# wangsibovictor/fora

Hardware: AMD Instinct MI355X
Metric: SSPPR queries/sec at eps=0.5 (higher is better)
Workload: dtype u64 fixed-point 2^-62 (f64 at the boundary)

## Files before the change

### fora_amd/csrc/fora_hip.hip

```cpp
#include "fora_kernels.h"
#include "fora_team.h"
#include "fora_bwd.h"
#include "../../include/fora_hip.h"

#include <algorithm>
#include <cmath>
#include <cstdio>
#include <cstdlib>
#include <cstring>
#include <string>
#include <vector>

using namespace fora;

struct fora_ctx;
static int build_hub_copy(fora_ctx *c, const int64_t *row_ptr, const int32_t *col);
static int build_quad_copies(fora_ctx *c);
namespace {

struct EvPair {
    hipEvent_t a, b;
    int kind;
};

// ... 16 lines not shown
    int64_t xb = 0, ax = 0, wx = 0;
    int64_t tail = -1;
    int64_t tail_always = 0;
    int64_t select_compact = -1;
    int64_t rounds = 1;
    int64_t round_div = 4;
    int64_t defer = 0;
    int64_t defer_min = 0;
    int64_t team = -1;
    int64_t team_size = 0;
    int64_t team_tail = -1;
    int64_t team_xcd = 1;
    int64_t team_max = 0;
    int64_t team_hubs = 1024;
    int64_t tail_hubs = 1;
    int64_t team_log = -1;
    int64_t slot_major = -1;
    int64_t acc_group = 0;
    int64_t team_abort_level = 0;
    int64_t team_timeout_ms = 500;
    int64_t team_coop = 0;
    int64_t topk_bk_div = 16;
    int64_t quads = 1;
    int64_t pipeline = 0;
    int64_t profile = 1;
    int64_t grid = 2048;
    int64_t bwd_lds_cap = BWD_CAP_DEFAULT;
    int64_t bwd_chunk = 0;
};
static const struct { const char *name; int64_t Tunables::*field; bool layout; } OPTIONS[] = {
    {"direct", &Tunables::direct, true}, {"force_wide", &Tunables::force_wide, true}, {"pass_bins", &Tunables::pass_bins, true},
    {"no_split", &Tunables::no_split, true}, {"no_compact", &Tunables::no_compact, false}, {"walk_dg", &Tunables::walk_dg, false}, {"dg_hubs", &Tunables::dg_hubs, false}, {"hubs", &Tunables::hubs, true}, {"hubs_wide", &Tunables::hubs_wide, true}, {"hub_min", &Tunables::hub_min, false}, {"bkcap", &Tunables::bkcap, true},
    {"ovcap", &Tunables::ovcap, true}, {"tiny", &Tunables::tiny, false}, {"xb", &Tunables::xb, false}, {"ax", &Tunables::ax, false},
    {"wx", &Tunables::wx, false}, {"tail", &Tunables::tail, false}, {"tail_always", &Tunables::tail_always, false},
    {"select_compact", &Tunables::select_compact, false}, {"pipeline", &Tunables::pipeline, false}, {"team", &Tunables::team, true}, {"team_size", &Tunables::team_size, true}, {"team_tail", &Tunables::team_tail, false}, {"team_xcd", &Tunables::team_xcd, false}, {"team_max", &Tunables::team_max, true}, {"team_hubs", &Tunables::team_hubs, true}, {"team_log", &Tunables::team_log, false}, {"topk_bk_div", &Tunables::topk_bk_div, true}, {"quads", &Tunables::quads, false}, {"team_timeout_ms", &Tunables::team_timeout_ms, false}, {"team_abort_level", &Tunables::team_abort_level, false}, {"acc_group", &Tunables::acc_group, false}, {"slot_major", &Tunables::slot_major, false}, {"team_coop", &Tunables::team_coop, false}, {"tail_hubs", &Tunables::tail_hubs, false}, {"rounds", &Tunables::rounds, false}, {"defer", &Tunables::defer, true}, {"defer_min", &Tunables::defer_min, false}, {"round_div", &Tunables::round_div, false},
    {"profile", &Tunables::profile, false}, {"grid", &Tunables::grid, false},
    {"bwd_lds_cap", &Tunables::bwd_lds_cap, false}, {"bwd_chunk", &Tunables::bwd_chunk, false},
};
static bool schedule_option(const char *name) {
    return !strcmp(name, "rounds") || !strcmp(name, "round_div") || !strcmp(name, "defer") || !strcmp(name, "defer_min");
}
static Tunables tunables_from_env() {
    Tunables t;
    for (const auto &o : OPTIONS) {
        if (schedule_option(o.name)) continue;
        std::string env = "FORA_HIP_";
        for (const char *p = o.name; *p; p++) env += (char)toupper((unsigned char)*p);
        if (const char *e = getenv(env.c_str())) if (*e) t.*(o.field) = atoll(e);
    }
    return t;
// ... 29 lines not shown
    uint32_t *d_dg_perm = nullptr, *d_dg_inv = nullptr, *d_dg_colp = nullptr, *d_dg_rec = nullptr, *d_dg_invb = nullptr;
    uint8_t *d_dg_T = nullptr;
    WalkDG dg{};
    uint32_t *d_colt = nullptr, *d_team_off = nullptr, *d_team_n2l = nullptr, *d_team_l2n = nullptr;
    uint32_t *d_team_hubtgt = nullptr;
    uint32_t team_H = 0, team_hubs_opt = 0;
    uint16_t *d_team_rlog_id = nullptr; uint64_t *d_team_rlog_val = nullptr; uint32_t team_rlog_cap = 0;
    uint64_t *d_team_rowl = nullptr, *d_team_rsvl = nullptr;
    uint16_t *d_team_deg16 = nullptr;
    uint32_t *d_team_rowq = nullptr;
    uint32_t team_T = 0, team_R = 0, team_force = 0;
    bool team_checked = false, team_wanted = false;
    double dangling_frac = 0;
    uint64_t team_cap = 0;
    uint32_t *d_team_msg = nullptr;
    uint64_t *d_team_inct = nullptr;
    unsigned long long *d_team_cnt = nullptr;
    uint32_t *d_team_ctl = nullptr;
    uint32_t team_n = 0;
    bool team_dirty = false;
    bool hub_for_team = false;
    bool team_timeout_seen = false;
    int team_suspend = 0;
    uint64_t team_fallbacks = 0;
    int team_fit = -1;
    bool team_coop_ok = false;
    bool team_coop_failed = false;

    bool have_params = false;
    double alpha = 0.2, epsilon = 0.5, rmax_scale = 1.0, rmax = 0, omega = 0;
// ... 126 lines not shown
void free_index(fora_ctx *c) {
    dfree(c->d_rw_idx); dfree(c->d_idx_off); dfree(c->d_idx_cnt);
    c->idx_len = 0; c->have_index = false;
}
void free_workspace(fora_ctx *c) {
    dfree(c->d_residue); dfree(c->d_ppr); dfree(c->d_wl[0]); dfree(c->d_wl[1]); dfree(c->d_scratch);
    dfree(c->d_counters); dfree(c->d_qs); dfree(c->d_src); dfree(c->d_err);
    dfree(c->d_ppr2); dfree(c->d_cursor); c->cursor_epoch = 0; dfree(c->d_active); dfree(c->d_above); dfree(c->d_sel_thr); dfree(c->d_topk_ids); dfree(c->d_topk_sc);
    dfree(c->d_upper); dfree(c->d_lower); dfree(c->d_filter); dfree(c->d_fail); dfree(c->d_round_walks);
    dfree(c->d_lb_sc); dfree(c->d_lb_ids); c->lb_cap = 0;
    dfree(c->d_nz_counts);
    c->topk_cap = 0;
    dfree(c->d_fl[0]); dfree(c->d_fl[1]); dfree(c->d_fl_count); dfree(c->d_inc_tab[0]); dfree(c->d_inc_tab[1]); dfree(c->d_ov_w); dfree(c->d_ov_inc); dfree(c->d_ov_count); dfree(c->d_ov_bin);
    dfree(c->d_bk_w); dfree(c->d_bk_inc); dfree(c->d_bk_count); dfree(c->d_wit_count); dfree(c->d_sw); dfree(c->d_tile_ctr);
    dfree(c->d_dbm); dfree(c->d_dflag); dfree(c->d_dl); dfree(c->d_hubsum);
    dfree(c->d_team_msg); dfree(c->d_team_inct); dfree(c->d_team_rsvl); dfree(c->d_team_rlog_id); dfree(c->d_team_rlog_val); dfree(c->d_team_cnt); dfree(c->d_team_ctl); c->team_n = 0; c->team_fit = -1;
    if (c->h_flc) (void)hipHostFree(c->h_flc);
    c->h_flc = nullptr;
    if (c->h_pinned) (void)hipHostFree(c->h_pinned);
    c->h_pinned = nullptr;
    if (c->h_qs_pin) (void)hipHostFree(c->h_qs_pin);
    c->h_qs_pin = nullptr;
    if (c->h_steps_pin) (void)hipHostFree(c->h_steps_pin);
    c->h_steps_pin = nullptr;
    c->B = 0;
    c->B_memcap = 0;
}

constexpr size_t N_COUNTERS = 2 * (size_t)(MAX_LEVELS + 2) + 2;
static uint32_t slab_grid_x(const fora_ctx *c, int nq) {
    const int64_t nchunk = ((int64_t)c->n + BLOCK - 1) / BLOCK;
// ... 224 lines not shown
               c->wit_cap >= pe.wits && c->bk_cap == pe.bk_cap && c->sub == pe.sub;
    };
    {
        int need = c->batch_req > 0 ? c->batch_req : std::min(want_slots > 0 ? want_slots : 1024, 1024);
        if (c->batch_req == 0 && c->B > 0 && c->B_memcap > 0) need = std::min(need, c->B_memcap);
        if (keepable(need)) { const WsPlan pe = plan_workspace(c, omega_hint, c->B); return ensure_row_split(c, pe.nbins, pe.pbins); }
    }
    int B = c->batch_req > 0 ? c->batch_req : 0;
    if (B == 0) {
        free_workspace(c);
        size_t fr = 0, tot = 0;
        HIPCHK(c, hipMemGetInfo(&fr, &tot));
        uint64_t budget = (uint64_t)(fr * (c->opt_.pipeline == 1 ? 0.4 : 0.75));
        if (c->team_T) {
            const uint64_t T = c->team_T, nt = std::max<uint64_t>(1, (uint64_t)c->prop.multiProcessorCount * TEAM_WGS_PER_CU / T);
            const uint64_t team_bytes = nt * (2 * c->team_cap * 4 + 3 * T * (c->team_R + 64 + c->team_H) * 8 + T * (10ull << 17) + 2 * T * T * 8);
            budget -= std::min<uint64_t>(budget / 2, team_bytes);
        }
        B = (int)std::min<uint64_t>(1024, std::max<uint64_t>(1, budget / p.per_slot));
    }
    B = std::max(1, B);
    const int memcap = B;
    if (want_slots > 0 && c->batch_req == 0) B = std::min(B, std::max(want_slots, 1));
    p = plan_workspace(c, omega_hint, B);
    const uint64_t scratch = (uint64_t)B * p.scratch;
    free_workspace(c);
    const uint64_t slab = (uint64_t)B * n;
    HIPCHK(c, hipMalloc(&c->d_residue, slab * 8));
    HIPCHK(c, hipMalloc(&c->d_ppr, slab * 8));
    if (p.binned) {
        HIPCHK(c, hipMalloc(&c->d_fl[0], slab * 4));
// ... 12 lines not shown
        HIPCHK(c, hipMalloc(&c->d_bk_count, (size_t)B * p.pbins * p.sub * 4));
        HIPCHK(c, hipHostMalloc(&c->h_flc, (size_t)FLC_RING * B * 4 * CSTRIDE));
        c->dbm_words = (uint32_t)((uint64_t)p.nbins << (bin_shift(c) - 6));
        HIPCHK(c, hipMalloc(&c->d_dbm, 2 * (size_t)B * c->dbm_words * 8));
        HIPCHK(c, hipMalloc(&c->d_dflag, 2 * (size_t)B * p.nbins * 4));
        if (c->opt_.defer > 0) HIPCHK(c, hipMalloc(&c->d_dl, 2 * slab * 4));
        if (c->hubs && c->hub_shift == bin_shift(c)) HIPCHK(c, hipMalloc(&c->d_hubsum, (size_t)B * p.sub * c->hubs * 8));
        if (c->team_T) {
            const uint32_t T = c->team_T;
            uint32_t nteams = std::max<uint32_t>(1, (uint32_t)c->prop.multiProcessorCount * TEAM_WGS_PER_CU / T);
            if (c->opt_.team_max > 0) nteams = std::min<uint32_t>(nteams, (uint32_t)c->opt_.team_max);
            size_t fr = 0, tot = 0;
            HIPCHK(c, hipMemGetInfo(&fr, &tot));
            c->team_rlog_cap = 1u << 17;
            auto per_team_bytes = [&](uint32_t logcap) {
                return 2 * c->team_cap * 4 + 3 * (uint64_t)T * (c->team_R + 64 + c->team_H) * 8 + (uint64_t)T * logcap * 10 + 2 * (uint64_t)T * T * 8;
            };
            while (c->team_rlog_cap > 1024 && per_team_bytes(c->team_rlog_cap) > fr / 4) c->team_rlog_cap /= 2;
            const uint64_t per_team = per_team_bytes(c->team_rlog_cap);
            nteams = (uint32_t)std::max<uint64_t>(1, std::min<uint64_t>(nteams, (uint64_t)(fr / 2) / std::max<uint64_t>(1, per_team)));
            HIPCHK(c, hipMalloc(&c->d_team_msg, (size_t)nteams * 2 * c->team_cap * 4 + 64 + diag::TEAM_MSG_PROBE_WORDS * 4));
            HIPCHK(c, hipMalloc(&c->d_team_inct, (size_t)nteams * 2 * T * (c->team_R + 64 + c->team_H) * 8));
            HIPCHK(c, hipMalloc(&c->d_team_rsvl, (size_t)nteams * T * c->team_R * 8));
            HIPCHK(c, hipMemset(c->d_team_rsvl, 0, (size_t)nteams * T * c->team_R * 8));
            HIPCHK(c, hipMalloc(&c->d_team_rlog_id, (size_t)nteams * T * c->team_rlog_cap * 2));
            HIPCHK(c, hipMalloc(&c->d_team_rlog_val, (size_t)nteams * T * c->team_rlog_cap * 8));
            HIPCHK(c, hipMalloc(&c->d_team_cnt, (size_t)nteams * 2 * T * T * 8));
            HIPCHK(c, hipMalloc(&c->d_team_ctl, (64 + (size_t)nteams * 5 * 16 * 2 + (size_t)nteams * ((size_t)B + 2)) * 4));
            c->team_n = nteams;
            if (int rf = team_fits(c)) return rf;
        }
    } else {
        HIPCHK(c, hipMalloc(&c->d_wl[0], slab * 8));
        HIPCHK(c, hipMalloc(&c->d_wl[1], slab * 8));
    }
    HIPCHK(c, hipMalloc(&c->d_scratch, scratch));
// ... 309 lines not shown
    if (hipOccupancyMaxActiveBlocksPerMultiprocessor(&per_cu, (const void *)k_push_team, TEAM_THREADS, lds) != hipSuccess) { (void)hipGetLastError(); per_cu = 0; }
    const uint32_t grid = c->team_n * c->team_T;
    c->team_fit = (uint64_t)per_cu * (uint64_t)c->prop.multiProcessorCount >= grid ? 1 : 0;
    int coop = 0;
    if (hipDeviceGetAttribute(&coop, hipDeviceAttributeCooperativeLaunch, c->device) != hipSuccess) { (void)hipGetLastError(); coop = 0; }
    c->team_coop_ok = c->opt_.team_coop == 1 && coop != 0;
    return FORA_OK;
}
int run_push_team(fora_ctx *c, const Dev &d) {
    const uint32_t T = c->team_T, nteams = c->team_n;
    TeamDev a{};
    a.n = d.n; a.nq = d.nq; a.rowinfo = d.rowinfo; a.row_ptr = d.row_ptr; a.deg = d.deg; a.src = d.src;
    a.residue = d.residue; a.ppr = d.ppr; a.fl0 = d.fl[0]; a.fl_count0 = d.fl_count[0]; a.inc_tab0 = d.inc_tab[0];
    a.segq_cap = d.segq_cap; a.qs = d.qs; a.err = d.err; a.afix = d.afix; a.t1 = d.t1;
    a.T = T; a.R = c->team_R; a.nteams = nteams;
    a.colt = c->d_colt; a.rowq = c->d_team_rowq; a.n2l = c->d_team_n2l; a.l2n = c->d_team_l2n; a.deg16 = c->d_team_deg16; a.rowl = c->d_team_rowl; a.rsvl = c->d_team_rsvl; a.rlog_id = c->d_team_rlog_id; a.rlog_val = c->d_team_rlog_val; a.rlog_cap = c->opt_.team_log == 0 ? 0u : c->opt_.team_log > 0 ? std::min<uint32_t>((uint32_t)c->opt_.team_log, c->team_rlog_cap) : c->team_rlog_cap; a.H = c->team_H; a.hubtgt = c->d_team_hubtgt; a.off = c->d_team_off; a.msg = c->d_team_msg; a.inct = c->d_team_inct; a.cntw = c->d_team_cnt;
    a.ctl = c->d_team_ctl;
    a.sync = (unsigned long long *)(c->d_team_ctl + 64);
    a.slot_seq = c->d_team_ctl + 64 + (size_t)nteams * 5 * 16 * 2;
    const int64_t tail_auto = 4096;
    a.tail_max = (uint32_t)std::min<int64_t>(std::max<int64_t>(c->opt_.team_tail < 0 ? tail_auto : c->opt_.team_tail, 0), 0x7FFFFFFF);
    if (c->opt_.tail == 0) a.tail_max = 0;
    a.tail_always = c->opt_.tail_always == 1 ? 1u : 0u;
    const uint32_t grid = nteams * T;
    a.xcd = (c->opt_.team_xcd >= 1 && grid % 8 == 0 && (grid / 8) % T == 0) ? (uint32_t)c->opt_.team_xcd : 0u;
    a.stamps = c->d_stamps;
    a.abort_level = (uint32_t)std::min<int64_t>(std::max<int64_t>(c->opt_.team_abort_level, 0), 1 << 20);
    a.timeout_ticks = (uint64_t)std::min<int64_t>(std::max<int64_t>(c->opt_.team_timeout_ms, 0), 60000) * 100000ull;
    const size_t lds = ((size_t)a.R + 1 + a.H) * 8;
    if (c->team_dirty) { HIPCHK(c, hipMemsetAsync(c->d_team_rsvl, 0, (size_t)nteams * T * c->team_R * 8, c->stream)); c->team_dirty = false; }
    HIPCHK(c, hipMemsetAsync(c->d_team_ctl, 0, (64 + (size_t)nteams * 5 * 16 * 2) * 4, c->stream));
    HIPCHK(c, hipMemsetAsync(c->d_team_cnt, 0, (size_t)nteams * 2 * T * T * 8, c->stream));
    HIPCHK(c, hipMemsetAsync(a.slot_seq, 0xFF, (size_t)nteams * ((size_t)d.nq + 2) * 4, c->stream));
    int h = ev_begin(c, 10);
    bool launched = false;
    if (c->team_coop_ok && !c->team_coop_failed) {
        void *args[] = {(void *)&a};
        const hipError_t le = hipLaunchCooperativeKernel((const void *)k_push_team, dim3(grid), dim3(TEAM_THREADS), args, (unsigned)lds, c->stream);
// ... 2003 lines not shown
```

### fora_amd/csrc/fora_team.h

```cpp
#pragma once
#include "fora_kernels.h"

namespace fora {

constexpr int TEAM_MAX = 32;
constexpr int TEAM_LBITS = 15;
#ifndef FORA_TEAM_THREADS
#define FORA_TEAM_THREADS 1024
#endif
constexpr int TEAM_THREADS = FORA_TEAM_THREADS;
#ifndef FORA_TEAM_WGS_PER_CU
#define FORA_TEAM_WGS_PER_CU (FORA_TEAM_THREADS == 1024 ? 1 : 2)
#endif
constexpr int TEAM_WGS_PER_CU = FORA_TEAM_WGS_PER_CU;
constexpr int TEAM_NW = TEAM_THREADS / 64;
constexpr uint32_t TEAM_R_CAP = TEAM_WGS_PER_CU == 1 ? 15296 : 7680;
constexpr int TEAM_NIT = (TEAM_R_CAP + TEAM_THREADS - 1) / TEAM_THREADS;
#ifndef FORA_TEAM_EPT
#define FORA_TEAM_EPT 4
#endif
#ifndef FORA_TEAM_CU
#define FORA_TEAM_CU 4
#endif
#ifndef FORA_TEAM_MPL
// ... 24 lines not shown
    uint32_t T, R, nteams;
    const uint32_t *colt;
    const uint32_t *rowq;
    const uint32_t *n2l;
    const uint32_t *l2n;
    const uint16_t *deg16;
    const uint64_t *rowl;
    uint64_t *rsvl;
    uint16_t *rlog_id;
    uint64_t *rlog_val;
    uint32_t rlog_cap;
    uint32_t H;
    const uint32_t *hubtgt;
    const uint32_t *off;
    uint32_t *msg;
    uint64_t *inct;
    unsigned long long *cntw;
    unsigned long long *sync;
    uint32_t *slot_seq;
    uint32_t *ctl;
    uint32_t tail_max;
    uint32_t tail_always;
    uint32_t xcd;
    unsigned long long *stamps;
    uint64_t timeout_ticks;
    uint32_t abort_level;
};

typedef const __attribute__((address_space(4))) TeamDev *TeamArgs;
__device__ __forceinline__ TeamArgs team_args() {
// ... 37 lines not shown


#ifndef FORA_TEAM_HEAVY
#define FORA_TEAM_HEAVY 1024
#endif
constexpr uint32_t TEAM_HEAVY = FORA_TEAM_HEAVY;
#ifndef FORA_TEAM_NHEAVY
#define FORA_TEAM_NHEAVY 128
#endif
#ifndef FORA_TEAM_MAXGROUPS
#define FORA_TEAM_MAXGROUPS 256
#endif
constexpr int TEAM_NHEAVY = FORA_TEAM_NHEAVY;
constexpr int TEAM_MAXGROUPS = FORA_TEAM_MAXGROUPS;

__device__ __forceinline__ void team_emit(const uint32_t (&word)[TEAM_EPT], const uint32_t (&dst)[TEAM_EPT], uint32_t *s_fill, uint32_t *mout) {
    uint32_t slot[TEAM_EPT];
#pragma unroll
    for (int k = 0; k < TEAM_EPT; k++) {
        slot[k] = 0;
        if (dst[k] != TEAM_EMPTY) slot[k] = atomicAdd(&s_fill[dst[k]], 1u);
    }
#pragma unroll
    for (int k = 0; k < TEAM_EPT; k++)
        if (dst[k] != TEAM_EMPTY) mout[slot[k]] = word[k];
    diag::team_emit_probe(word, dst, slot, mout, TEAM_EMPTY);
}

__global__ void __launch_bounds__(TEAM_THREADS, TEAM_THREADS * TEAM_WGS_PER_CU / 256) k_push_team(const TeamDev kernarg_only) {
    extern __shared__ uint64_t res[];
    __shared__ uint16_t w_list[TEAM_NW][128];
    __shared__ unsigned long long s_gmask[TEAM_MAXGROUPS];
    __shared__ uint32_t h_ent[TEAM_NHEAVY], h_ebeg[TEAM_NHEAVY], h_deg[TEAM_NHEAVY], h_cstart[TEAM_NHEAVY];
    __shared__ uint8_t w_mark[TEAM_NW][64] __attribute__((aligned(4)));
    __shared__ uint64_t w_inc[TEAM_NW][64];
    __shared__ uint64_t h_inc[TEAM_NHEAVY];
    __shared__ uint32_t s_hubent;
    __shared__ uint32_t s_hchunks, s_hnext, s_wdone;
    __shared__ uint32_t s_fill[TEAM_MAX], s_moff[TEAM_MAX];
    __shared__ uint32_t s_slot, s_F, s_ok, s_ncross, s_nheavy, s_gnext, s_abort, s_rsvovf;
    __shared__ unsigned long long s_dang, s_acc[3];
    (void)kernarg_only;

    uint32_t T, R, H, team, me, cap_total, coffv;
    const int tid0 = threadIdx.x;
    const int tid = tid0, lane = tid & 63, wid = tid >> 6;
    uint32_t dgp[(TEAM_NIT + 1) / 2], thh[TEAM_NIT];
    bool same_xcd;
    uint32_t hub_tg0;
    {
        const TeamArgs a = team_args();
        T = a->T; R = a->R; H = a->H;
        hub_tg0 = (uint32_t)tid0 < H ? a->hubtgt[tid0] : 0u;
        if (a->xcd) {
            const uint32_t x = blockIdx.x & 7u, j = blockIdx.x >> 3, per = gridDim.x >> 3;
// ... 85 lines not shown
        }
        uint64_t acc_res = 0, acc_pops = 0, acc_relax = 0;
        uint32_t peak = 0, nlev = 0;
        uint32_t logbase = 0;
        bool final_round = false;
        if (fresh(tid0) == 0) s_rsvovf = 0;

        TSTAMP_LEVEL_DECL
        for (uint32_t L = 0;; L++) {
            const int tid = fresh(tid0), lane = tid & 63, wid = __builtin_amdgcn_readfirstlane(tid >> 6);
            if (L > 0) {
                const TeamArgs a = team_args();
                const uint32_t par = (g - 1) & 1u;
                const uint32_t *min_ = a->msg + ((uint64_t)team * 2 + par) * cap_total;
                const uint64_t *tin = a->inct + ((uint64_t)team * 2 + par) * T * tstride;
                const uint32_t tagp = g & 0xFFFFFFu;
                const unsigned long long *cwin = a->cntw + ((uint64_t)team * 2 + par) * T * T + (uint64_t)me * T;
                const unsigned long long full = T >= 64 ? ~0ull : (1ull << T) - 1ull;
                unsigned long long donemask = 0;
                uint32_t fsum = 0, spins = 0;
                uint64_t w_t0 = 0;
                while (donemask != full) {
                unsigned long long wv = 0;
                if ((uint32_t)lane < T) wv = __hip_atomic_load(&cwin[lane], __ATOMIC_RELAXED, __HIP_MEMORY_SCOPE_AGENT);
                const unsigned long long ready = __ballot((uint32_t)lane < T && (uint32_t)(wv >> 40) == tagp) & ~donemask;
                if (!ready) {
                    TSTAMP_SLEEP(8, 2, 40);
                    if ((++spins & 255u) == 0) {
                        const TeamArgs ar = team_args();
                        uint32_t *ctl = ar->ctl;
// ... 1 lines not shown
                        if (w_t0 == 0) w_t0 = now;
                        bool stop = __hip_atomic_load(&ctl[32], __ATOMIC_RELAXED, __HIP_MEMORY_SCOPE_AGENT) != 0;
                        if (!stop && now - w_t0 > ar->timeout_ticks) {
                            __hip_atomic_store(&ctl[32], 1u, __ATOMIC_RELAXED, __HIP_MEMORY_SCOPE_AGENT);
                            if (lane == 0) atomicOr(ar->err, ERR_TEAM_TIMEOUT);
                            stop = true;
                        }
                        if (stop) { if (lane == 0) s_abort = 1u; break; }
                    }
                    continue;
                }
                if (!same_xcd) { __builtin_amdgcn_fence(__ATOMIC_ACQUIRE, "agent"); asm volatile("s_waitcnt vmcnt(0)" ::: "memory"); }
                donemask |= ready;
                const bool mine = (ready >> lane) & 1ull;
                const uint32_t c = mine ? (uint32_t)wv & 0xFFFFFFu : 0u;
                fsum += mine ? (uint32_t)(wv >> 24) & 0xFFFFu : 0u;
                constexpr int MPL = FORA_TEAM_MPL, SEGSH = MPL == 4 ? 8 : 7;
                constexpr int CU = MPL == 4 ? (FORA_TEAM_CU + 1) / 2 : FORA_TEAM_CU;
                const uint32_t ns = (c + (1u << SEGSH) - 1u) >> SEGSH;
                const uint32_t r0 = ((uint32_t)wid + 2u * TEAM_NW - (uint32_t)lane % TEAM_NW) % TEAM_NW;
                const uint32_t kmine = ns > r0 ? (ns - r0 + TEAM_NW - 1) / TEAM_NW : 0u;
                uint32_t nmine;
                const uint32_t pmine = wave_excl_scan(kmine, nmine);
                for (uint32_t i0 = 0; i0 < nmine; i0 += CU) {
                    uint32_t mw[CU][MPL];
                    uint4 mq[CU];
                    uint32_t srcm[CU], left[CU];
                    const uint32_t *mp[CU];
#pragma unroll
                    for (int k = 0; k < CU; k++) {
                        const bool have = i0 + k < nmine;
                        const uint32_t ic = have ? i0 + k : 0u;
                        const uint32_t sidx = (uint32_t)__popcll(__ballot(pmine <= ic)) - 1u;
                        const uint32_t j = (uint32_t)__builtin_amdgcn_readlane((int)r0, (int)sidx) + (ic - (uint32_t)__builtin_amdgcn_readlane((int)pmine, (int)sidx)) * TEAM_NW;
                        const uint32_t n_s = (uint32_t)__builtin_amdgcn_readlane((int)c, (int)sidx);
                        const uint32_t idx = (j << SEGSH) + (uint32_t)MPL * lane;
                        left[k] = (have && idx < n_s) ? n_s - idx : 0u;
                        srcm[k] = sidx;
                        mp[k] = min_ + (uint64_t)(uint32_t)__builtin_amdgcn_readlane((int)coffv, (int)sidx) + (left[k] ? idx : 0u);
                        if (MPL != 4) {
                            const unsigned long long mm = __hip_atomic_load((const unsigned long long *)mp[k], __ATOMIC_RELAXED, __HIP_MEMORY_SCOPE_AGENT);
                            mw[k][0] = (uint32_t)mm; mw[k][1] = (uint32_t)(mm >> 32);
                        }
                    }
                    if (MPL == 4) {
                        static_assert(MPL != 4 || CU <= 2, "one asm statement per trip");
                        if (CU == 1) asm volatile("global_load_dwordx4 %0, %1, off sc1\n\ts_waitcnt vmcnt(0)" : "=&v"(mq[0]) : "v"(mp[0]) : "memory");
                        else asm volatile("global_load_dwordx4 %0, %2, off sc1\n\tglobal_load_dwordx4 %1, %3, off sc1\n\ts_waitcnt vmcnt(0)"
                                          : "=&v"(mq[0]), "=&v"(mq[CU - 1]) : "v"(mp[0]), "v"(mp[CU - 1]) : "memory");
#pragma unroll
                        for (int k = 0; k < CU; k++) { mw[k][0] = mq[k].x; mw[k][1] = mq[k].y; mw[k][MPL - 2] = mq[k].z; mw[k][MPL - 1] = mq[k].w; }
                    }
                    uint64_t vv[CU][MPL];
#pragma unroll
                    for (int k = 0; k < CU; k++) {
                        const uint64_t *tb = tin + (uint64_t)srcm[k] * tstride;
#pragma unroll
                        for (int u = 0; u < MPL; u++)
                            vv[k][u] = __hip_atomic_load((const unsigned long long *)&tb[left[k] > (uint32_t)u ? (mw[k][u] >> TEAM_LBITS) : 0u], __ATOMIC_RELAXED, __HIP_MEMORY_SCOPE_AGENT);
                    }
#pragma unroll
                    for (int k = 0; k < CU; k++)
#pragma unroll
                        for (int u = 0; u < MPL; u++)
                            vv[k][u] += diag::team_gather_probe(tin + (uint64_t)srcm[k] * tstride, mw[k][u] >> TEAM_LBITS, left[k] > (uint32_t)u);
#pragma unroll
                    for (int k = 0; k < CU; k++)
#pragma unroll
                        for (int u = 0; u < MPL; u++)
                            if (left[k] > (uint32_t)u && vv[k][u]) atomicAdd((unsigned long long *)&res[mw[k][u] & TEAM_LMASK], (unsigned long long)vv[k][u]);
// ... 9 lines not shown
                const TeamArgs af = team_args();
                bool quit = s_abort != 0;
                if (af->abort_level && L == af->abort_level) {
                    if (tid == 0) { __hip_atomic_store(&af->ctl[32], 1u, __ATOMIC_RELAXED, __HIP_MEMORY_SCOPE_AGENT); atomicOr(af->err, ERR_TEAM_TIMEOUT); }
                    quit = true;
                }
                if (quit) return;
                const uint32_t F = s_F;
                if (F) nlev++;
                peak = max(peak, F);
                const uint32_t tail_max = af->tail_max;
                final_round = F == 0 || (tail_max && F <= tail_max && (peak > tail_max || af->tail_always));
            }
            uint32_t crossmask = 0;
            if (tid < TEAM_MAX) s_fill[tid] = s_moff[tid];
            if (tid == 0) { s_dang = 0; s_ncross = 0; s_nheavy = 0; s_gnext = 0; s_hchunks = 0; s_hnext = 0; s_wdone = 0; s_hubent = 0; }
            if (tid < TEAM_NHEAVY) h_deg[tid] = 0;
            if (L > 0) {
                const TeamArgs a = team_args();
                const uint64_t t1 = a->t1;
                const bool thr_small = (t1 >> 47) == 0;
                const uint32_t t1_lo = (uint32_t)t1, t1_hi = (uint32_t)(t1 >> 32);
                constexpr int SG = 5;
#pragma unroll
                for (int g0 = 0; g0 < TEAM_NIT; g0 += SG) {
                    if ((uint32_t)g0 * TEAM_THREADS + (uint32_t)wid * 64u < R) {
                        uint64_t r[SG];
#pragma unroll
                        for (int k = 0; k < SG; k++) {
                            const uint32_t l = (g0 + k) * TEAM_THREADS + tid;
                            r[k] = ((uint32_t)(g0 + k) * TEAM_THREADS + (uint32_t)wid * 64u < R) ? res[l] : 0ull;
                        }
#pragma unroll
                        for (int k = 0; k < SG; k++) {
                            const int it = g0 + k;
                            if ((uint32_t)it * TEAM_THREADS + (uint32_t)wid * 64u < R) {
                                bool c = false;
                                const uint32_t rhi = (uint32_t)(r[k] >> 32);
// ... 1 lines not shown
                                else if (rhi == thh[it] && r[k]) {
                                    uint32_t dg = (dgp[it >> 1] >> ((it & 1) * 16)) & 0xFFFFu;
                                    asm volatile("" : "+v"(dg));
                                    if (dg == 0xFFFFu) {
                                        uint32_t li = it * TEAM_THREADS + tid;
                                        asm volatile("" : "+v"(li));
                                        const TeamArgs ar = team_args();
                                        c = r[k] >= node_thr(t1, ar->deg[ar->l2n[(uint64_t)me * R + li]]);
                                    }
                                    else if (thr_small) c = r[k] >= (uint64_t)t1_lo * dg + ((uint64_t)(t1_hi * dg) << 32);
                                    else c = r[k] >= node_thr(t1, dg);
                                }
                                if (c) crossmask |= 1u << it;
                                const unsigned long long mk = __ballot(c);
                                if (lane == 0) s_gmask[it * TEAM_NW + wid] = mk;
                            }
                        }
                    }
                }
                if (tid == 0) {
                    const uint64_t rs = res[R];
                    s_gmask[ngroups - 1] = (me == src_owner && rs && rs >= node_thr(t1, src_deg)) ? 1ull : 0ull;
                }
            } else if (me == src_owner && tid == 0) {
                res[src_local] = FIX_ONE;
            }
            TSTAMP(1);
            __syncthreads();
            if (final_round) {
                const TeamArgs a = team_args();
                const uint32_t n = (uint32_t)a->n;
                const uint32_t *l2n = a->l2n + (uint64_t)me * R;
                uint32_t *fl0 = a->fl0 + slab;
                uint64_t *inc0 = a->inc_tab0 + (uint64_t)q * a->segq_cap;
                uint64_t *residue = a->residue + slab;
                uint32_t mine = 0;
                for (uint32_t it = 0; it < nit; it++) mine += (uint32_t)__popcll(__ballot((crossmask >> it) & 1u));
                const bool spare = wid == 0 && s_gmask[ngroups - 1] != 0;
// ... 76 lines not shown
                    }
#pragma unroll
                    for (int it = 0; it < TEAM_NIT; it++) {
                        if ((uint32_t)it * TEAM_THREADS + (uint32_t)wid * 64u < R) {
                            const uint32_t l = it * TEAM_THREADS + tid;
                            uint64_t rs = res[l];
                            if (ovf) { const uint64_t o = rsvl[l]; if (o) { rs += o; rsvl[l] = 0; } }
                            if (rs) { ppr[lv[it]] = rs; res[l] = 0; }
                        }
                    }
                }
                TSTAMP(6);
                break;
            }
            uint64_t my_dang = 0;
            {
                const TeamArgs a = team_args();
                uint32_t *mout = a->msg + ((uint64_t)team * 2 + (g & 1u)) * cap_total;
                uint64_t *tout = a->inct + (((uint64_t)team * 2 + (g & 1u)) * T + me) * tstride;
                const uint64_t *rowl = a->rowl + (uint64_t)me * R;
                const uint32_t rlog_cap = a->rlog_cap;
                uint16_t *rlog_id = a->rlog_id + ((uint64_t)team * T + me) * rlog_cap;
                uint64_t *rlog_val = a->rlog_val + ((uint64_t)team * T + me) * rlog_cap;
                const uint64_t afix = a->afix;
                const uint32_t *colt = a->colt;
                uint16_t *list = w_list[wid];
                uint64_t *winc = w_inc[wid];
                uint8_t *mark = w_mark[wid];
                uint32_t npend = 0, gcur = 0, gend = 0;
                bool drained = false;
                constexpr uint32_t bsz = 64;
                if (L == 0) { drained = true; if (me == src_owner && wid == 0) { if (lane == 0) list[0] = (uint16_t)src_local; npend = 1; } }
                for (;;) {
// ... 33 lines not shown
                        const uint64_t rr = res[l];
                        res[l] = 0;
                        uint32_t deg = spare ? src_deg : (uint32_t)(rw >> 19) & 8191u;
                        if (!spare && deg == 8191u) deg = team_args()->deg[(uint32_t)rw & 0x7FFFFu];
                        uint64_t rsv_add, dang;
                        const uint64_t inc = pop_value(afix, rr, deg, rsv_add, dang);
                        if (logi < rlog_cap) { rlog_val[logi] = direct ? 0ull : rsv_add; rlog_id[logi] = direct ? (uint16_t)0 : (uint16_t)l; }
                        if (direct && rsv_add) {
                            const TeamArgs ar = team_args();
                            if (spare) ar->ppr[slab + src] = rsv_old + rsv_add;
                            else { (ar->rsvl + ((uint64_t)team * T + me) * R)[l] = rsv_old + rsv_add; s_rsvovf = 1u; }
                        }
                        acc_res += rsv_add; my_dang += dang; acc_pops++; acc_relax += deg;
                        ebeg = spare ? srcq : (uint32_t)(rw >> 32);
                        cnt = inc ? deg : 0u;
                        if (cnt) tout[ebase + lane] = inc;
                        winc[lane] = inc;
                        if (cnt > TEAM_HEAVY) {
                            const uint32_t hi = atomicAdd(&s_nheavy, 1u);
                            if (hi < (uint32_t)TEAM_NHEAVY) {
                                h_ent[hi] = ebase + lane; h_ebeg[hi] = ebeg; h_inc[hi] = inc;
                                h_cstart[hi] = atomicAdd(&s_hchunks, (cnt + TEAM_CHUNK - 1) / TEAM_CHUNK);
                                __atomic_store_n(&h_deg[hi], cnt, __ATOMIC_RELEASE);
                                cnt = 0;
                            }
                        }
                    }
                    if (npend > 64) {
                        const uint16_t keep = list[64 + (lane < 63 ? lane : 63)];
                        __builtin_amdgcn_wave_barrier();
                        if ((uint32_t)lane < npend - 64) list[lane] = keep;
// ... 22 lines not shown
                        const uint32_t rb = (uint32_t)__shfl((int)rowbase, (int)si);
                        uint4 w4 = colt4[q < total ? rb + q : 0u];
                        if (q >= total) w4 = make_uint4(TEAM_EMPTY, TEAM_EMPTY, TEAM_EMPTY, TEAM_EMPTY);
                        const uint32_t w[TEAM_EPT] = {w4.x, w4.y, w4.z, w4.w};
                        const uint32_t entw = (ebase + si) << TEAM_LBITS;
                        uint32_t word[TEAM_EPT], dst[TEAM_EPT];
#pragma unroll
                        for (int k = 0; k < TEAM_EPT; k++) {
                            dst[k] = w[k] == TEAM_EMPTY ? TEAM_EMPTY : w[k] >> TEAM_LBITS;
                            word[k] = (w[k] & TEAM_LMASK) | entw;
                            if (w[k] != TEAM_EMPTY && (w[k] & 0x80000000u)) {
                                atomicAdd(&s_hub[w[k] & 0x7FFFFFFFu], (unsigned long long)winc[si]);
                                dst[k] = TEAM_EMPTY;
                            }
                        }
                        team_emit(word, dst, s_fill, mout);
                    }
                    TSTAMP(3);
                }
            }
            TSTAMP(2);
            my_dang = wave_sum(my_dang);
            if (lane == 0 && my_dang) atomicAdd(&s_dang, (unsigned long long)my_dang);
            {
                if (lane == 0) atomicAdd(&s_wdone, 1u);
                for (;;) {
                    uint32_t k = TEAM_EMPTY, fin = 0;
                    if (lane == 0) {
                        const uint32_t nx = __atomic_load_n(&s_hnext, __ATOMIC_RELAXED), tot = __atomic_load_n(&s_hchunks, __ATOMIC_RELAXED);
                        if (nx < tot) { if (atomicCAS(&s_hnext, nx, nx + 1u) == nx) k = nx; }
                        else if (__atomic_load_n(&s_wdone, __ATOMIC_RELAXED) == (uint32_t)TEAM_NW && nx >= __atomic_load_n(&s_hchunks, __ATOMIC_RELAXED)) fin = 1;
                    }
                    k = (uint32_t)__builtin_amdgcn_readfirstlane((int)k);
                    fin = (uint32_t)__builtin_amdgcn_readfirstlane((int)fin);
                    if (fin) break;
                    if (k == TEAM_EMPTY) { TSTAMP_SLEEP(9, 1, 30); continue; }
                    const TeamArgs a = team_args();
                    uint32_t *mout = a->msg + ((uint64_t)team * 2 + (g & 1u)) * cap_total;
                    const uint32_t *colt = a->colt;
                    uint32_t eb = 0, dgh = 0, ent = 0, c0 = 0;
                    uint64_t hinc = 0;
                    for (bool found = false; !found;) {
                        const uint32_t nh = min(__atomic_load_n(&s_nheavy, __ATOMIC_RELAXED), (uint32_t)TEAM_NHEAVY);
                        for (uint32_t hb = 0; hb < nh && !found; hb += 64) {
                            const uint32_t h = hb + lane;
                            const uint32_t dg = h < nh ? __atomic_load_n(&h_deg[h], __ATOMIC_ACQUIRE) : 0u;
                            const uint32_t cs = dg ? h_cstart[h] : 0u;
                            const unsigned long long hit = __ballot(dg && k >= cs && k < cs + (dg + TEAM_CHUNK - 1) / TEAM_CHUNK);
                            if (hit) {
                                const uint32_t hs = hb + (uint32_t)__ffsll((long long)hit) - 1u;
                                eb = h_ebeg[hs]; dgh = h_deg[hs]; ent = h_ent[hs] << TEAM_LBITS; hinc = h_inc[hs]; c0 = (k - h_cstart[hs]) * TEAM_CHUNK;
                                found = true;
                            }
// ... 2 lines not shown
                    uint32_t word[TEAM_EPT], dst[TEAM_EPT];
                    {
                        const uint32_t q = (c0 >> 2) + lane;
                        uint4 w4 = make_uint4(TEAM_EMPTY, TEAM_EMPTY, TEAM_EMPTY, TEAM_EMPTY);
                        if (q < ((dgh + 3u) >> 2)) w4 = ((const uint4 *)colt)[(uint64_t)eb + q];
                        const uint32_t w[TEAM_EPT] = {w4.x, w4.y, w4.z, w4.w};
#pragma unroll
                        for (int kk = 0; kk < TEAM_EPT; kk++) {
                            dst[kk] = TEAM_EMPTY; word[kk] = 0;
                            if (w[kk] != TEAM_EMPTY) {
                                if (w[kk] & 0x80000000u) atomicAdd(&s_hub[w[kk] & 0x7FFFFFFFu], (unsigned long long)hinc);
                                else { dst[kk] = w[kk] >> TEAM_LBITS; word[kk] = (w[kk] & TEAM_LMASK) | ent; }
                            }
                        }
                    }
                    team_emit(word, dst, s_fill, mout);
                }
            }
            TSTAMP(6);
            __syncthreads();
            TSTAMP(7);
            {
                const TeamArgs a = team_args();
                uint32_t *mout = a->msg + ((uint64_t)team * 2 + (g & 1u)) * cap_total;
                uint64_t *tout = a->inct + (((uint64_t)team * 2 + (g & 1u)) * T + me) * tstride;
                if (tid == 0 && s_dang) {
                    const uint32_t ent = s_ncross, pos = atomicAdd(&s_fill[src_owner], 1u);
                    tout[ent] = s_dang;
                    mout[pos] = src_local | (ent << TEAM_LBITS);
                }
                if ((uint32_t)tid < H) {
                    const uint32_t *hubtgt = a->hubtgt;
                    for (uint32_t h = tid; h < H; h += TEAM_THREADS) {
                        const unsigned long long hv = s_hub[h];
                        if (hv) {
                            s_hub[h] = 0;
                            const uint32_t tg = h < (uint32_t)TEAM_THREADS ? hub_tg0 : hubtgt[h], ent = s_ncross + 1 + atomicAdd(&s_hubent, 1u);
                            tout[ent] = hv;
                            mout[atomicAdd(&s_fill[tg >> TEAM_LBITS], 1u)] = (tg & TEAM_LMASK) | (ent << TEAM_LBITS);
                        }
                    }
                }
                asm volatile("s_waitcnt vmcnt(0)" ::: "memory");
                __syncthreads();
                const uint32_t tag = (g + 1u) & 0xFFFFFFu;
                if (!same_xcd) {
                    if (tid == 0) { __builtin_amdgcn_fence(__ATOMIC_RELEASE, "agent"); asm volatile("s_waitcnt vmcnt(0)" ::: "memory"); }
                    __syncthreads();
                }
                if ((uint32_t)tid < T) {
                    unsigned long long *cw = team_args()->cntw + ((uint64_t)team * 2 + (g & 1u)) * T * T;
                    __hip_atomic_store(&cw[(uint32_t)tid * T + me], (unsigned long long)(s_fill[tid] - s_moff[tid]) | ((unsigned long long)s_ncross << 24) | ((unsigned long long)tag << 40),
                                       __ATOMIC_RELAXED, __HIP_MEMORY_SCOPE_AGENT);
                }
// ... 31 lines not shown
```

Before: 6757.

## Inline message values for small frontiers in team push exchange

Adds a parallel 64-bit value array beside each team message buffer. When the number of pushing nodes in a level is at or below a threshold (default 256), senders write the increment directly next to each message and receivers read it from there, instead of going through the per-sender increment table indirection. The aim is to cut the dependent gather on the receive side for sparse levels, at the cost of extra 8-byte writes per message and larger team buffers that shrink the slot budget.

```diff
diff --git a/fora_amd/csrc/fora_hip.hip b/fora_amd/csrc/fora_hip.hip
--- a/fora_amd/csrc/fora_hip.hip
+++ b/fora_amd/csrc/fora_hip.hip
@@ -54,6 +54,7 @@
     int64_t team_max = 0;
     int64_t team_hubs = 1024;
     int64_t tail_hubs = 1;
+    int64_t team_inline = -1;
     int64_t team_log = -1;
     int64_t slot_major = -1;
     int64_t acc_group = 0;
@@ -73,7 +74,7 @@
     {"no_split", &Tunables::no_split, true}, {"no_compact", &Tunables::no_compact, false}, {"walk_dg", &Tunables::walk_dg, false}, {"dg_hubs", &Tunables::dg_hubs, false}, {"hubs", &Tunables::hubs, true}, {"hubs_wide", &Tunables::hubs_wide, true}, {"hub_min", &Tunables::hub_min, false}, {"bkcap", &Tunables::bkcap, true},
     {"ovcap", &Tunables::ovcap, true}, {"tiny", &Tunables::tiny, false}, {"xb", &Tunables::xb, false}, {"ax", &Tunables::ax, false},
     {"wx", &Tunables::wx, false}, {"tail", &Tunables::tail, false}, {"tail_always", &Tunables::tail_always, false},
-    {"select_compact", &Tunables::select_compact, false}, {"pipeline", &Tunables::pipeline, false}, {"team", &Tunables::team, true}, {"team_size", &Tunables::team_size, true}, {"team_tail", &Tunables::team_tail, false}, {"team_xcd", &Tunables::team_xcd, false}, {"team_max", &Tunables::team_max, true}, {"team_hubs", &Tunables::team_hubs, true}, {"team_log", &Tunables::team_log, false}, {"topk_bk_div", &Tunables::topk_bk_div, true}, {"quads", &Tunables::quads, false}, {"team_timeout_ms", &Tunables::team_timeout_ms, false}, {"team_abort_level", &Tunables::team_abort_level, false}, {"acc_group", &Tunables::acc_group, false}, {"slot_major", &Tunables::slot_major, false}, {"team_coop", &Tunables::team_coop, false}, {"tail_hubs", &Tunables::tail_hubs, false}, {"rounds", &Tunables::rounds, false}, {"defer", &Tunables::defer, true}, {"defer_min", &Tunables::defer_min, false}, {"round_div", &Tunables::round_div, false},
+    {"select_compact", &Tunables::select_compact, false}, {"pipeline", &Tunables::pipeline, false}, {"team", &Tunables::team, true}, {"team_size", &Tunables::team_size, true}, {"team_tail", &Tunables::team_tail, false}, {"team_xcd", &Tunables::team_xcd, false}, {"team_max", &Tunables::team_max, true}, {"team_hubs", &Tunables::team_hubs, true}, {"team_log", &Tunables::team_log, false}, {"team_inline", &Tunables::team_inline, false}, {"topk_bk_div", &Tunables::topk_bk_div, true}, {"quads", &Tunables::quads, false}, {"team_timeout_ms", &Tunables::team_timeout_ms, false}, {"team_abort_level", &Tunables::team_abort_level, false}, {"acc_group", &Tunables::acc_group, false}, {"slot_major", &Tunables::slot_major, false}, {"team_coop", &Tunables::team_coop, false}, {"tail_hubs", &Tunables::tail_hubs, false}, {"rounds", &Tunables::rounds, false}, {"defer", &Tunables::defer, true}, {"defer_min", &Tunables::defer_min, false}, {"round_div", &Tunables::round_div, false},
     {"profile", &Tunables::profile, false}, {"grid", &Tunables::grid, false},
     {"bwd_lds_cap", &Tunables::bwd_lds_cap, false}, {"bwd_chunk", &Tunables::bwd_chunk, false},
 };
@@ -133,6 +134,7 @@
     double dangling_frac = 0;
     uint64_t team_cap = 0;
     uint32_t *d_team_msg = nullptr;
+    uint64_t *d_team_msgv = nullptr;
     uint64_t *d_team_inct = nullptr;
     unsigned long long *d_team_cnt = nullptr;
     uint32_t *d_team_ctl = nullptr;
@@ -289,7 +291,7 @@
     dfree(c->d_fl[0]); dfree(c->d_fl[1]); dfree(c->d_fl_count); dfree(c->d_inc_tab[0]); dfree(c->d_inc_tab[1]); dfree(c->d_ov_w); dfree(c->d_ov_inc); dfree(c->d_ov_count); dfree(c->d_ov_bin);
     dfree(c->d_bk_w); dfree(c->d_bk_inc); dfree(c->d_bk_count); dfree(c->d_wit_count); dfree(c->d_sw); dfree(c->d_tile_ctr);
     dfree(c->d_dbm); dfree(c->d_dflag); dfree(c->d_dl); dfree(c->d_hubsum);
-    dfree(c->d_team_msg); dfree(c->d_team_inct); dfree(c->d_team_rsvl); dfree(c->d_team_rlog_id); dfree(c->d_team_rlog_val); dfree(c->d_team_cnt); dfree(c->d_team_ctl); c->team_n = 0; c->team_fit = -1;
+    dfree(c->d_team_msg); dfree(c->d_team_msgv); dfree(c->d_team_inct); dfree(c->d_team_rsvl); dfree(c->d_team_rlog_id); dfree(c->d_team_rlog_val); dfree(c->d_team_cnt); dfree(c->d_team_ctl); c->team_n = 0; c->team_fit = -1;
     if (c->h_flc) (void)hipHostFree(c->h_flc);
     c->h_flc = nullptr;
     if (c->h_pinned) (void)hipHostFree(c->h_pinned);
@@ -544,7 +546,7 @@
         uint64_t budget = (uint64_t)(fr * (c->opt_.pipeline == 1 ? 0.4 : 0.75));
         if (c->team_T) {
             const uint64_t T = c->team_T, nt = std::max<uint64_t>(1, (uint64_t)c->prop.multiProcessorCount * TEAM_WGS_PER_CU / T);
-            const uint64_t team_bytes = nt * (2 * c->team_cap * 4 + 3 * T * (c->team_R + 64 + c->team_H) * 8 + T * (10ull << 17) + 2 * T * T * 8);
+            const uint64_t team_bytes = nt * (2 * c->team_cap * 12 + 3 * T * (c->team_R + 64 + c->team_H) * 8 + T * (10ull << 17) + 2 * T * T * 8);
             budget -= std::min<uint64_t>(budget / 2, team_bytes);
         }
         B = (int)std::min<uint64_t>(1024, std::max<uint64_t>(1, budget / p.per_slot));
@@ -587,12 +589,13 @@
             HIPCHK(c, hipMemGetInfo(&fr, &tot));
             c->team_rlog_cap = 1u << 17;
             auto per_team_bytes = [&](uint32_t logcap) {
-                return 2 * c->team_cap * 4 + 3 * (uint64_t)T * (c->team_R + 64 + c->team_H) * 8 + (uint64_t)T * logcap * 10 + 2 * (uint64_t)T * T * 8;
+                return 2 * c->team_cap * 12 + 3 * (uint64_t)T * (c->team_R + 64 + c->team_H) * 8 + (uint64_t)T * logcap * 10 + 2 * (uint64_t)T * T * 8;
             };
             while (c->team_rlog_cap > 1024 && per_team_bytes(c->team_rlog_cap) > fr / 4) c->team_rlog_cap /= 2;
             const uint64_t per_team = per_team_bytes(c->team_rlog_cap);
             nteams = (uint32_t)std::max<uint64_t>(1, std::min<uint64_t>(nteams, (uint64_t)(fr / 2) / std::max<uint64_t>(1, per_team)));
             HIPCHK(c, hipMalloc(&c->d_team_msg, (size_t)nteams * 2 * c->team_cap * 4 + 64 + diag::TEAM_MSG_PROBE_WORDS * 4));
+            HIPCHK(c, hipMalloc(&c->d_team_msgv, (size_t)nteams * 2 * c->team_cap * 8 + 64));
             HIPCHK(c, hipMalloc(&c->d_team_inct, (size_t)nteams * 2 * T * (c->team_R + 64 + c->team_H) * 8));
             HIPCHK(c, hipMalloc(&c->d_team_rsvl, (size_t)nteams * T * c->team_R * 8));
             HIPCHK(c, hipMemset(c->d_team_rsvl, 0, (size_t)nteams * T * c->team_R * 8));
@@ -932,7 +935,7 @@
     a.residue = d.residue; a.ppr = d.ppr; a.fl0 = d.fl[0]; a.fl_count0 = d.fl_count[0]; a.inc_tab0 = d.inc_tab[0];
     a.segq_cap = d.segq_cap; a.qs = d.qs; a.err = d.err; a.afix = d.afix; a.t1 = d.t1;
     a.T = T; a.R = c->team_R; a.nteams = nteams;
-    a.colt = c->d_colt; a.rowq = c->d_team_rowq; a.n2l = c->d_team_n2l; a.l2n = c->d_team_l2n; a.deg16 = c->d_team_deg16; a.rowl = c->d_team_rowl; a.rsvl = c->d_team_rsvl; a.rlog_id = c->d_team_rlog_id; a.rlog_val = c->d_team_rlog_val; a.rlog_cap = c->opt_.team_log == 0 ? 0u : c->opt_.team_log > 0 ? std::min<uint32_t>((uint32_t)c->opt_.team_log, c->team_rlog_cap) : c->team_rlog_cap; a.H = c->team_H; a.hubtgt = c->d_team_hubtgt; a.off = c->d_team_off; a.msg = c->d_team_msg; a.inct = c->d_team_inct; a.cntw = c->d_team_cnt;
+    a.colt = c->d_colt; a.rowq = c->d_team_rowq; a.n2l = c->d_team_n2l; a.l2n = c->d_team_l2n; a.deg16 = c->d_team_deg16; a.rowl = c->d_team_rowl; a.rsvl = c->d_team_rsvl; a.rlog_id = c->d_team_rlog_id; a.rlog_val = c->d_team_rlog_val; a.rlog_cap = c->opt_.team_log == 0 ? 0u : c->opt_.team_log > 0 ? std::min<uint32_t>((uint32_t)c->opt_.team_log, c->team_rlog_cap) : c->team_rlog_cap; a.H = c->team_H; a.hubtgt = c->d_team_hubtgt; a.off = c->d_team_off; a.msg = c->d_team_msg; a.msgv = c->d_team_msgv; a.inct = c->d_team_inct; a.cntw = c->d_team_cnt;
     a.ctl = c->d_team_ctl;
     a.sync = (unsigned long long *)(c->d_team_ctl + 64);
     a.slot_seq = c->d_team_ctl + 64 + (size_t)nteams * 5 * 16 * 2;
@@ -940,6 +943,7 @@
     a.tail_max = (uint32_t)std::min<int64_t>(std::max<int64_t>(c->opt_.team_tail < 0 ? tail_auto : c->opt_.team_tail, 0), 0x7FFFFFFF);
     if (c->opt_.tail == 0) a.tail_max = 0;
     a.tail_always = c->opt_.tail_always == 1 ? 1u : 0u;
+    a.inl_max = (uint32_t)std::min<int64_t>(c->opt_.team_inline < 0 ? 256 : c->opt_.team_inline, 0xFFFF);
     const uint32_t grid = nteams * T;
     a.xcd = (c->opt_.team_xcd >= 1 && grid % 8 == 0 && (grid / 8) % T == 0) ? (uint32_t)c->opt_.team_xcd : 0u;
     a.stamps = c->d_stamps;
diff --git a/fora_amd/csrc/fora_team.h b/fora_amd/csrc/fora_team.h
--- a/fora_amd/csrc/fora_team.h
+++ b/fora_amd/csrc/fora_team.h
@@ -62,6 +62,8 @@
     const uint32_t *hubtgt;
     const uint32_t *off;
     uint32_t *msg;
+    uint64_t *msgv;
+    uint32_t inl_max;
     uint64_t *inct;
     unsigned long long *cntw;
     unsigned long long *sync;
@@ -129,7 +131,8 @@
 constexpr int TEAM_NHEAVY = FORA_TEAM_NHEAVY;
 constexpr int TEAM_MAXGROUPS = FORA_TEAM_MAXGROUPS;
 
-__device__ __forceinline__ void team_emit(const uint32_t (&word)[TEAM_EPT], const uint32_t (&dst)[TEAM_EPT], uint32_t *s_fill, uint32_t *mout) {
+__device__ __forceinline__ void team_emit(const uint32_t (&word)[TEAM_EPT], const uint32_t (&dst)[TEAM_EPT], uint32_t *s_fill, uint32_t *mout,
+                                          uint64_t *vout, uint64_t val) {
     uint32_t slot[TEAM_EPT];
 #pragma unroll
     for (int k = 0; k < TEAM_EPT; k++) {
@@ -138,7 +141,10 @@
     }
 #pragma unroll
     for (int k = 0; k < TEAM_EPT; k++)
-        if (dst[k] != TEAM_EMPTY) mout[slot[k]] = word[k];
+        if (dst[k] != TEAM_EMPTY) {
+            mout[slot[k]] = word[k];
+            if (vout) vout[slot[k]] = val;
+        }
     diag::team_emit_probe(word, dst, slot, mout, TEAM_EMPTY);
 }
 
@@ -154,6 +160,7 @@
     __shared__ uint32_t s_hchunks, s_hnext, s_wdone;
     __shared__ uint32_t s_fill[TEAM_MAX], s_moff[TEAM_MAX];
     __shared__ uint32_t s_slot, s_F, s_ok, s_ncross, s_nheavy, s_gnext, s_abort, s_rsvovf;
+    __shared__ uint32_t s_npop[2];
     __shared__ unsigned long long s_dang, s_acc[3];
     (void)kernarg_only;
 
@@ -269,6 +276,8 @@
                 const uint32_t par = (g - 1) & 1u;
                 const uint32_t *min_ = a->msg + ((uint64_t)team * 2 + par) * cap_total;
                 const uint64_t *tin = a->inct + ((uint64_t)team * 2 + par) * T * tstride;
+                const uint64_t *vin = a->msgv + ((uint64_t)team * 2 + par) * cap_total;
+                const uint32_t inl_max = a->inl_max;
                 const uint32_t tagp = g & 0xFFFFFFu;
                 const unsigned long long *cwin = a->cntw + ((uint64_t)team * 2 + par) * T * T + (uint64_t)me * T;
                 const unsigned long long full = T >= 64 ? ~0ull : (1ull << T) - 1ull;
@@ -300,7 +309,8 @@
                 donemask |= ready;
                 const bool mine = (ready >> lane) & 1ull;
                 const uint32_t c = mine ? (uint32_t)wv & 0xFFFFFFu : 0u;
-                fsum += mine ? (uint32_t)(wv >> 24) & 0xFFFFu : 0u;
+                const uint32_t spops = mine ? (uint32_t)(wv >> 24) & 0xFFFFu : 0u;
+                fsum += spops;
                 constexpr int MPL = FORA_TEAM_MPL, SEGSH = MPL == 4 ? 8 : 7;
                 constexpr int CU = MPL == 4 ? (FORA_TEAM_CU + 1) / 2 : FORA_TEAM_CU;
                 const uint32_t ns = (c + (1u << SEGSH) - 1u) >> SEGSH;
@@ -311,7 +321,8 @@
                 for (uint32_t i0 = 0; i0 < nmine; i0 += CU) {
                     uint32_t mw[CU][MPL];
                     uint4 mq[CU];
-                    uint32_t srcm[CU], left[CU];
+                    uint32_t srcm[CU], left[CU], mo[CU];
+                    bool inl[CU];
                     const uint32_t *mp[CU];
 #pragma unroll
                     for (int k = 0; k < CU; k++) {
@@ -323,11 +334,14 @@
                         const uint32_t idx = (j << SEGSH) + (uint32_t)MPL * lane;
                         left[k] = (have && idx < n_s) ? n_s - idx : 0u;
                         srcm[k] = sidx;
-                        mp[k] = min_ + (uint64_t)(uint32_t)__builtin_amdgcn_readlane((int)coffv, (int)sidx) + (left[k] ? idx : 0u);
+                        mo[k] = (uint32_t)__builtin_amdgcn_readlane((int)coffv, (int)sidx) + (left[k] ? idx : 0u);
+                        mp[k] = min_ + (uint64_t)mo[k];
                         if (MPL != 4) {
                             const unsigned long long mm = __hip_atomic_load((const unsigned long long *)mp[k], __ATOMIC_RELAXED, __HIP_MEMORY_SCOPE_AGENT);
                             mw[k][0] = (uint32_t)mm; mw[k][1] = (uint32_t)(mm >> 32);
                         }
+                        const uint32_t sp = (uint32_t)__builtin_amdgcn_readlane((int)spops, (int)sidx);
+                        inl[k] = inl_max != 0 && sp <= inl_max;
                     }
                     if (MPL == 4) {
                         static_assert(MPL != 4 || CU <= 2, "one asm statement per trip");
@@ -340,6 +354,12 @@
                     uint64_t vv[CU][MPL];
 #pragma unroll
                     for (int k = 0; k < CU; k++) {
+                        if (inl[k]) {
+#pragma unroll
+                            for (int u = 0; u < MPL; u++)
+                                vv[k][u] = __hip_atomic_load((const unsigned long long *)&vin[mo[k] + (uint32_t)u], __ATOMIC_RELAXED, __HIP_MEMORY_SCOPE_AGENT);
+                            continue;
+                        }
                         const uint64_t *tb = tin + (uint64_t)srcm[k] * tstride;
 #pragma unroll
                         for (int u = 0; u < MPL; u++)
@@ -379,7 +399,7 @@
             }
             uint32_t crossmask = 0;
             if (tid < TEAM_MAX) s_fill[tid] = s_moff[tid];
-            if (tid == 0) { s_dang = 0; s_ncross = 0; s_nheavy = 0; s_gnext = 0; s_hchunks = 0; s_hnext = 0; s_wdone = 0; s_hubent = 0; }
+            if (tid == 0) { s_dang = 0; s_ncross = 0; s_nheavy = 0; s_gnext = 0; s_hchunks = 0; s_hnext = 0; s_wdone = 0; s_hubent = 0; s_npop[(L + 1) & 1] = 0; }
             if (tid < TEAM_NHEAVY) h_deg[tid] = 0;
             if (L > 0) {
                 const TeamArgs a = team_args();
@@ -387,6 +407,7 @@
                 const bool thr_small = (t1 >> 47) == 0;
                 const uint32_t t1_lo = (uint32_t)t1, t1_hi = (uint32_t)(t1 >> 32);
                 constexpr int SG = 5;
+                uint32_t npw = 0;
 #pragma unroll
                 for (int g0 = 0; g0 < TEAM_NIT; g0 += SG) {
                     if ((uint32_t)g0 * TEAM_THREADS + (uint32_t)wid * 64u < R) {
@@ -418,14 +439,18 @@
                                 if (c) crossmask |= 1u << it;
                                 const unsigned long long mk = __ballot(c);
                                 if (lane == 0) s_gmask[it * TEAM_NW + wid] = mk;
+                                npw += (uint32_t)__popcll(mk);
                             }
                         }
                     }
                 }
                 if (tid == 0) {
                     const uint64_t rs = res[R];
-                    s_gmask[ngroups - 1] = (me == src_owner && rs && rs >= node_thr(t1, src_deg)) ? 1ull : 0ull;
-                }
+                    const bool cs = me == src_owner && rs && rs >= node_thr(t1, src_deg);
+                    s_gmask[ngroups - 1] = cs ? 1ull : 0ull;
+                    if (cs) npw++;
+                }
+                if (lane == 0 && npw) atomicAdd(&s_npop[L & 1], npw);
             } else if (me == src_owner && tid == 0) {
                 res[src_local] = FIX_ONE;
             }
@@ -532,9 +557,16 @@
                 break;
             }
             uint64_t my_dang = 0;
+            bool inl;
+            {
+                const uint32_t npop = L == 0 ? (me == src_owner ? 1u : 0u) : s_npop[L & 1];
+                const uint32_t im = team_args()->inl_max;
+                inl = im != 0 && npop <= im;
+            }
             {
                 const TeamArgs a = team_args();
                 uint32_t *mout = a->msg + ((uint64_t)team * 2 + (g & 1u)) * cap_total;
+                uint64_t *vout = inl ? a->msgv + ((uint64_t)team * 2 + (g & 1u)) * cap_total : nullptr;
                 uint64_t *tout = a->inct + (((uint64_t)team * 2 + (g & 1u)) * T + me) * tstride;
                 const uint64_t *rowl = a->rowl + (uint64_t)me * R;
                 const uint32_t rlog_cap = a->rlog_cap;
@@ -598,7 +630,7 @@
                         acc_res += rsv_add; my_dang += dang; acc_pops++; acc_relax += deg;
                         ebeg = spare ? srcq : (uint32_t)(rw >> 32);
                         cnt = inc ? deg : 0u;
-                        if (cnt) tout[ebase + lane] = inc;
+                        if (cnt && !inl) tout[ebase + lane] = inc;
                         winc[lane] = inc;
                         if (cnt > TEAM_HEAVY) {
                             const uint32_t hi = atomicAdd(&s_nheavy, 1u);
@@ -651,7 +683,7 @@
                                 dst[k] = TEAM_EMPTY;
                             }
                         }
-                        team_emit(word, dst, s_fill, mout);
+                        team_emit(word, dst, s_fill, mout, vout, vout ? winc[si] : 0ull);
                     }
                     TSTAMP(3);
                 }
@@ -674,6 +706,7 @@
                     if (k == TEAM_EMPTY) { TSTAMP_SLEEP(9, 1, 30); continue; }
                     const TeamArgs a = team_args();
                     uint32_t *mout = a->msg + ((uint64_t)team * 2 + (g & 1u)) * cap_total;
+                    uint64_t *vout = inl ? a->msgv + ((uint64_t)team * 2 + (g & 1u)) * cap_total : nullptr;
                     const uint32_t *colt = a->colt;
                     uint32_t eb = 0, dgh = 0, ent = 0, c0 = 0;
                     uint64_t hinc = 0;
@@ -706,7 +739,7 @@
                             }
                         }
                     }
-                    team_emit(word, dst, s_fill, mout);
+                    team_emit(word, dst, s_fill, mout, vout, hinc);
                 }
             }
             TSTAMP(6);
@@ -716,9 +749,10 @@
                 const TeamArgs a = team_args();
                 uint32_t *mout = a->msg + ((uint64_t)team * 2 + (g & 1u)) * cap_total;
                 uint64_t *tout = a->inct + (((uint64_t)team * 2 + (g & 1u)) * T + me) * tstride;
+                uint64_t *vout = a->msgv + ((uint64_t)team * 2 + (g & 1u)) * cap_total;
                 if (tid == 0 && s_dang) {
                     const uint32_t ent = s_ncross, pos = atomicAdd(&s_fill[src_owner], 1u);
-                    tout[ent] = s_dang;
+                    if (inl) vout[pos] = s_dang; else tout[ent] = s_dang;
                     mout[pos] = src_local | (ent << TEAM_LBITS);
                 }
                 if ((uint32_t)tid < H) {
@@ -728,8 +762,9 @@
                         if (hv) {
                             s_hub[h] = 0;
                             const uint32_t tg = h < (uint32_t)TEAM_THREADS ? hub_tg0 : hubtgt[h], ent = s_ncross + 1 + atomicAdd(&s_hubent, 1u);
-                            tout[ent] = hv;
-                            mout[atomicAdd(&s_fill[tg >> TEAM_LBITS], 1u)] = (tg & TEAM_LMASK) | (ent << TEAM_LBITS);
+                            const uint32_t pos = atomicAdd(&s_fill[tg >> TEAM_LBITS], 1u);
+                            if (inl) vout[pos] = hv; else tout[ent] = hv;
+                            mout[pos] = (tg & TEAM_LMASK) | (ent << TEAM_LBITS);
                         }
                     }
                 }
```

Result: slower. 6685 (median of 2 runs) (-1.1%).
